# tanwanirahul/surreal

Hardware: AMD Instinct MI355X
Metric: PPO learner env-steps/sec/node (GAE+update) at 1/2/4/8 GPUs; % HBM roofline (higher is better)
Workload: dtype f32; 1 GPU; C3: synthetic PPO learner batch, reference PPO defaults (LSTM 100, horizon 5, heads 300x200, n_step 25, adapt, z-filter, 10/10 epochs), SawyerLift state dims (obs 42, act 8), 1024 segments split over 1 GPU(s) (1024 per GPU); segments_per_gpu=1024, n_step=25, env_steps_per_learn_per_gpu=25600, global_segments=1024, parallelism=single, epochs_run_last=10, ppo_mode=adapt, launch=hipGraph replay

## Files before the change

### surreal_amd/csrc/head_kernels.hip

```cpp
#include "smi_device.hpp"
#include "smi_internal.hpp"
#include "pol_rows.hpp"

namespace smi {

constexpr int HC_MAXK = 512;

struct HeadFwdArgs {
  const float* X; int64_t ldx; int K0;
  const float* W1; const float* b1;
  const float* W2; const float* b2;
  const float* W3; const float* b3;
  int h1, h2, out, tanh_out;
  float* HA1; float* HA2;
  float* Y; int64_t ldy;
  float* W1T; float* W2T;
  int64_t rows; const int* skip;
  int ld0, ld1, ld2;
  int o1, oR, shared;
  const float* vret; float* vgrad; float vscale;
  double* vpart;
};

struct HeadBwdArgs {
  const float* dZ; int out;
  const float* W3;
  const float* W2T;
  const float* W1T;
  int h1, h2, dx0, dxn;
  const float* HA1; const float* HA2;
  float* dH2; float* dH1;
  float* dX; int64_t lddx;
  const float* mask; int64_t ldm;
  int64_t rows; const int* skip;
  int ld2, ld1;
  PolRowArgs pg;
};

#ifdef SMI_PROF
__device__ unsigned long long g_head_ticks[2][10];
#define HEAD_T0() unsigned long long h_t0_ = wall_clock64(), h_prev_ = h_t0_
#define HEAD_TICK(k, id)                                                   \
  do {                                                                      \
    if (threadIdx.x == 0) {                                                 \
      const unsigned long long n_ = wall_clock64();                         \
      atomicAdd(&g_head_ticks[k][id], n_ - h_prev_);                        \
      h_prev_ = n_;                                                         \
    }                                                                       \
  } while (0)
#define HEAD_END(k)                                                        \
  do {                                                                      \
    if (threadIdx.x == 0) {                                                 \
      atomicAdd(&g_head_ticks[k][8], 1ull);                                 \
      atomicAdd(&g_head_ticks[k][9], wall_clock64() - h_t0_);               \
    }                                                                       \
  } while (0)
#else
#define HEAD_T0() (void)0
#define HEAD_TICK(k, id) (void)0
#define HEAD_END(k) (void)0
#endif

__device__ __forceinline__ void hc_sync() {
  __builtin_amdgcn_fence(__ATOMIC_RELEASE, "workgroup", "local");
  __builtin_amdgcn_s_barrier();
  __builtin_amdgcn_fence(__ATOMIC_ACQUIRE, "workgroup", "local");
}

constexpr int HC_D = 2;
constexpr int HC_XB = 4;
static_assert(HC_D >= 2, "ring of at least two chunks");
template <int NT>
struct HcStream {
  const float* wp[NT];
  float4 b[HC_D][NT];
  int K, nch, c0, cst, ntv;
  __device__ __forceinline__ void ldb(int c, float4 (&bb)[NT]) {
    const int lk = (threadIdx.x & 63) >> 4;
    const int kk = min(16 * c + 4 * lk, K - 4);
#pragma unroll
    for (int t = 0; t < NT; ++t) bb[t] = *reinterpret_cast<const float4*>(wp[t] + kk);
  }
  __device__ __forceinline__ void init(const float* __restrict__ W, int64_t ldw, int K_, int N,
                                       int nt0, int ntst, int c0_, int cst_) {
    const int li = threadIdx.x & 15;
    const int CT = (N + 15) >> 4;
    K = K_; nch = (K + 15) >> 4; c0 = c0_; cst = cst_;
    ntv = __builtin_amdgcn_readfirstlane(nt0 < CT ? (CT - 1 - nt0) / ntst + 1 : 0);
#pragma unroll
    for (int t = 0; t < NT; ++t) {
      const int n = min(16 * (nt0 + ntst * t) + li, N - 1);
      wp[t] = W + (int64_t)n * ldw;
    }
    ldb(min(c0, nch - 1), b[0]);
    ldb(min(c0 + cst, nch - 1), b[1]);
  }
};

template <int NT, int RT, bool CM = false>
__device__ __forceinline__ void hc_run(HcStream<NT>& S, const float* sA, int lda,
                                       f32x4 (&acc)[RT][NT]) {
  const int lane = threadIdx.x & 63, li = lane & 15, lk = lane >> 4;
#pragma unroll
  for (int rt = 0; rt < RT; ++rt)
#pragma unroll
    for (int t = 0; t < NT; ++t) acc[rt][t] = f32x4{0.f, 0.f, 0.f, 0.f};
  if (S.ntv == 0) return;
  const float* ap = sA + li * lda + 4 * lk;
  auto mm = [&](const float4 (&a)[RT], const float4 (&bb)[NT]) {
    if constexpr (!CM) {
#pragma unroll
      for (int t = 0; t < NT; ++t) {
#pragma unroll
        for (int rt = 0; rt < RT; ++rt) acc[rt][t] = mfma4(a[rt].x, bb[t].x, acc[rt][t]);
#pragma unroll
        for (int rt = 0; rt < RT; ++rt) acc[rt][t] = mfma4(a[rt].y, bb[t].y, acc[rt][t]);
#pragma unroll
        for (int rt = 0; rt < RT; ++rt) acc[rt][t] = mfma4(a[rt].z, bb[t].z, acc[rt][t]);
#pragma unroll
        for (int rt = 0; rt < RT; ++rt) acc[rt][t] = mfma4(a[rt].w, bb[t].w, acc[rt][t]);
      }
    } else {
#pragma unroll
      for (int t = 0; t < NT; ++t)
#pragma unroll
        for (int rt = 0; rt < RT; ++rt) acc[rt][t] = mfma4(a[rt].x, bb[t].x, acc[rt][t]);
#pragma unroll
      for (int t = 0; t < NT; ++t)
#pragma unroll
        for (int rt = 0; rt < RT; ++rt) acc[rt][t] = mfma4(a[rt].y, bb[t].y, acc[rt][t]);
#pragma unroll
      for (int t = 0; t < NT; ++t)
#pragma unroll
        for (int rt = 0; rt < RT; ++rt) acc[rt][t] = mfma4(a[rt].z, bb[t].z, acc[rt][t]);
#pragma unroll
      for (int t = 0; t < NT; ++t)
#pragma unroll
        for (int rt = 0; rt < RT; ++rt) acc[rt][t] = mfma4(a[rt].w, bb[t].w, acc[rt][t]);
    }
  };
  auto lda_ = [&](int c, float4 (&o)[RT]) {
#pragma unroll
    for (int rt = 0; rt < RT; ++rt)
      o[rt] = *reinterpret_cast<const float4*>(ap + rt * 16 * lda + 16 * c);
  };
  const int nch = S.nch, cst = S.cst, cl = nch - 1;
  int c = S.c0;
  float4 a[HC_D][RT];
#pragma unroll
  for (int d = 2; d < HC_D; ++d) S.ldb(min(c + d * cst, cl), S.b[d]);
#pragma unroll
  for (int d = 0; d < HC_D; ++d) lda_(min(c + d * cst, cl), a[d]);
  for (; c + (2 * HC_D - 1) * cst < nch; c += HC_D * cst) {
#pragma unroll
    for (int d = 0; d < HC_D; ++d) {
      mm(a[d], S.b[d]);
      lda_(c + (d + HC_D) * cst, a[d]);
      S.ldb(c + (d + HC_D) * cst, S.b[d]);
      __builtin_amdgcn_sched_barrier(0);
    }
  }
#pragma unroll
  for (int d = 0; d < HC_D; ++d) {
    if (c + d * cst < nch) mm(a[d], S.b[d]);
    lda_(min(c + (d + HC_D) * cst, cl), a[d]);
    S.ldb(min(c + (d + HC_D) * cst, cl), S.b[d]);
  }
#pragma unroll
  for (int d = 0; d < HC_D; ++d)
    if (c + (d + HC_D) * cst < nch) mm(a[d], S.b[d]);
}

template <int NT, int EPI, int RT>
__device__ __forceinline__ void hc_epi_load(int nt0, int N, const float* bias, const float* mask,
                                            int64_t r0, int64_t rows, float (&e)[RT][NT][4]) {
  const int lane = threadIdx.x & 63, li = lane & 15, lk = lane >> 4;
#pragma unroll
  for (int t = 0; t < NT; ++t) {
    const int nc = min(16 * (nt0 + 4 * t) + li, N - 1);
    if constexpr (EPI == 0) {
      e[0][t][0] = bias[nc];
    } else {
#pragma unroll
      for (int rt = 0; rt < RT; ++rt)
#pragma unroll
        for (int i = 0; i < 4; ++i) {
          const int64_t r = r0 + 16 * rt + 4 * lk + i;
          e[rt][t][i] = mask[(r < rows ? r : rows - 1) * N + nc];
        }
    }
  }
}

template <int NT, int EPI, int RT>
__device__ __forceinline__ void hc_store(const f32x4 (&acc)[RT][NT], const float (&e)[RT][NT][4],
                                         int nt0, int N, float* sO, int ldo) {
  const int lane = threadIdx.x & 63, li = lane & 15, lk = lane >> 4;
  const int CT = (N + 15) >> 4;
#pragma unroll
  for (int t = 0; t < NT; ++t) {
    const int nt = nt0 + 4 * t;
    if (nt >= CT) break;
    const int n = 16 * nt + li;
    const bool nv = n < N;
#pragma unroll
    for (int rt = 0; rt < RT; ++rt)
#pragma unroll
      for (int i = 0; i < 4; ++i) {
        const int r = 16 * rt + 4 * lk + i;
        float v;
        if constexpr (EPI == 0) {
          v = acc[rt][t][i] + e[0][t][0];
          v = v > 0.f ? v : 0.f;
        } else {
          v = e[rt][t][i] > 0.f ? acc[rt][t][i] : 0.f;
        }
        sO[r * ldo + n] = nv ? v : 0.f;
      }
  }
}

template <int RT>
__device__ __forceinline__ void hc_copy_out(const float* sO, int ld, int N, float* __restrict__ G,
                                           int64_t r0, int64_t rows) {
  if (G == nullptr) return;
  constexpr int J = HC_MAXK / 4 / 16;
  const int nq = N >> 2, q0 = threadIdx.x & 15;
#pragma unroll
  for (int rt = 0; rt < RT; ++rt) {
    const int r = (threadIdx.x >> 4) + 16 * rt;
    float4 v[J];
#pragma unroll
    for (int j = 0; j < J; ++j) {
      const int q = q0 + 16 * j;
      v[j] = q < nq ? *reinterpret_cast<const float4*>(sO + r * ld + 4 * q) : float4{0.f, 0.f, 0.f, 0.f};
    }
    if (r0 + r >= rows) continue;
    float* g = G + (r0 + r) * N;
#pragma unroll
    for (int j = 0; j < J; ++j) {
      const int q = q0 + 16 * j;
      if (q < nq) *reinterpret_cast<float4*>(g + 4 * q) = v[j];
    }
  }
}

__device__ __forceinline__ void hc_transpose_tile(const float* __restrict__ W, int M, int K,
                                                  float* __restrict__ WT, int tix, float* sT) {
  const int tk = (K + 31) >> 5;
  const int m0 = (tix / tk) * 32, k0 = (tix % tk) * 32;
  __syncthreads();
  static_assert(32 * 32 % kWG == 0, "whole tile passes");
  constexpr int TP = 32 * 32 / kWG;
  float v[TP];
#pragma unroll
  for (int i = 0; i < TP; ++i) {
    const int e = threadIdx.x + i * kWG, r = e >> 5, c = e & 31;
    v[i] = W[(int64_t)min(m0 + r, M - 1) * K + min(k0 + c, K - 1)];
  }
#pragma unroll
  for (int i = 0; i < TP; ++i) asm volatile("" : "+v"(v[i]));
#pragma unroll
  for (int i = 0; i < TP; ++i) {
    const int e = threadIdx.x + i * kWG, r = e >> 5, c = e & 31;
    if (m0 + r < M && k0 + c < K) sT[r * 33 + c] = v[i];
  }
  __syncthreads();
  for (int e = threadIdx.x; e < 32 * 32; e += kWG) {
    const int r = e >> 5, c = e & 31;
    if (k0 + r < K && m0 + c < M) WT[(int64_t)(k0 + r) * M + m0 + c] = sT[c * 33 + r];
  }
}

template <int NT1, int NT2, int RT>
__global__ void __launch_bounds__(kWG)
head_fwd_kernel(HeadFwdArgs a) {
  if (a.skip && a.skip[0] != 0) return;
  constexpr int R = HC_R * RT;
  extern __shared__ __attribute__((aligned(16))) float hsm[];
  float* s0 = hsm;
  float* s2 = hsm;
  float* s1 = hsm + a.o1;
  float* sR = hsm + a.oR;
  const int wave = __builtin_amdgcn_readfirstlane(threadIdx.x >> 6);
  const int lane = threadIdx.x & 63, li = lane & 15, lk = lane >> 4;
  const int64_t r0 = (int64_t)blockIdx.x * R;
  HEAD_T0();
  if (r0 < a.rows) {
    HcStream<NT1> S1;
    S1.init(a.W1, a.K0, a.K0, a.h1, wave, 4, 0, 1);
    float e1[RT][NT1][4];
    hc_epi_load<NT1, 0, RT>(wave, a.h1, a.b1, nullptr, r0, a.rows, e1);
    const int q0 = (a.ld0 - 4) >> 2;
    for (int e0 = threadIdx.x; e0 < R * q0; e0 += HC_XB * kWG) {
      f32x4 v[HC_XB];
#pragma unroll
      for (int k = 0; k < HC_XB; ++k) {
        const int e = min(e0 + k * kWG, R * q0 - 1);
        const int r = e / q0, q = e - r * q0;
        const int64_t rr = r0 + r < a.rows ? r0 + r : a.rows - 1;
        v[k] = *reinterpret_cast<const f32x4*>(a.X + rr * a.ldx + min(4 * q, a.K0 - 4));
      }
#pragma unroll
      for (int k = 0; k < HC_XB; ++k) {
        const int e = e0 + k * kWG;
        if (e >= R * q0) break;
        const int r = e / q0, q = e - r * q0;
        const f32x4 z = {0.f, 0.f, 0.f, 0.f};
        *reinterpret_cast<f32x4*>(s0 + r * a.ld0 + 4 * q) = 4 * q < a.K0 ? v[k] : z;
      }
    }
    __syncthreads();
    HEAD_TICK(0, 0);
    HcStream<NT2> S2;
    float e2[RT][NT2][4];
    {
      f32x4 acc[RT][NT1];
      __builtin_amdgcn_s_waitcnt(0x0F70);
      hc_run<NT1, RT>(S1, s0, a.ld0, acc);
      HEAD_TICK(0, 1);
      S2.init(a.W2, a.h1, a.h1, a.h2, wave, 4, 0, 1);
      hc_epi_load<NT2, 0, RT>(wave, a.h2, a.b2, nullptr, r0, a.rows, e2);
      if constexpr (RT == 2) {
        if (a.shared) hc_sync();
      }
      hc_store<NT1, 0, RT>(acc, e1, wave, a.h1, s1, a.ld1);
    }
    hc_sync();
    HEAD_TICK(0, 2);
    hc_copy_out<RT>(s1, a.ld1, a.h1, a.HA1, r0, a.rows);
    HEAD_TICK(0, 3);
    HcStream<1> S3;
    {
      f32x4 acc[RT][NT2];
      hc_run<NT2, RT>(S2, s1, a.ld1, acc);
      HEAD_TICK(0, 4);
      S3.init(a.W3, a.h2, a.h2, a.out, 0, 1, wave, 4);
      if constexpr (RT == 2) {
        if (a.shared) hc_sync();
      }
      hc_store<NT2, 0, RT>(acc, e2, wave, a.h2, s2, a.ld2);
    }
    hc_sync();
    HEAD_TICK(0, 5);
    hc_copy_out<RT>(s2, a.ld2, a.h2, a.HA2, r0, a.rows);
    {
      const float bn = a.b3[li < a.out ? li : a.out - 1];
      float vr[RT][4];
      if (a.vgrad) {
#pragma unroll
        for (int rt = 0; rt < RT; ++rt)
#pragma unroll
          for (int i = 0; i < 4; ++i)
            vr[rt][i] = a.vret[min(r0 + 16 * rt + 4 * lk + i, a.rows - 1)];
      }
      f32x4 acc[RT][1];
      hc_run<1, RT>(S3, s2, a.ld2, acc);
#pragma unroll
      for (int rt = 0; rt < RT; ++rt)
        *reinterpret_cast<float4*>(sR + ((wave * RT + rt) * 64 + lane) * 4) =
            float4{acc[rt][0][0], acc[rt][0][1], acc[rt][0][2], acc[rt][0][3]};
      hc_sync();
      double vs[5] = {0.0, 0.0, 0.0, 0.0, 0.0};
      if (wave == 0 && li < a.out) {
        __builtin_amdgcn_s_waitcnt(0x0F70);
#pragma unroll
        for (int rt = 0; rt < RT; ++rt)
#pragma unroll
          for (int i = 0; i < 4; ++i) {
            const int r = 16 * rt + 4 * lk + i;
            if (r0 + r >= a.rows) continue;
            const float v = ((sR[((0 * RT + rt) * 64 + lane) * 4 + i] + sR[((1 * RT + rt) * 64 + lane) * 4 + i]) +
                             (sR[((2 * RT + rt) * 64 + lane) * 4 + i] + sR[((3 * RT + rt) * 64 + lane) * 4 + i])) + bn;
            const float y = a.tanh_out ? tanhf(v) : v;
            a.Y[(r0 + r) * a.ldy + li] = y;
            if (a.vgrad) {
              const float rv = vr[rt][i];
              a.vgrad[r0 + r] = a.vscale * (y - rv);
              if (a.vpart) {
                const float e = y - rv;
                const double dd = (double)rv - (double)y;
                vs[0] += (double)(e * e);
                vs[1] += dd; vs[2] += dd * dd;
                vs[3] += (double)rv; vs[4] += (double)rv * (double)rv;
              }
            }
          }
      }
      if (a.vpart && wave == 0) {
#pragma unroll
        for (int k = 0; k < 5; ++k) {
          const double t = wave_sum_d(vs[k]);
          if (lane == 0) a.vpart[(int64_t)blockIdx.x * 5 + k] = t;
        }
      }
    }
  }
  HEAD_TICK(0, 6);
  if (a.W1T) {
    const int t1 = ((a.h1 + 31) >> 5) * ((a.K0 + 31) >> 5);
    const int t2 = ((a.h2 + 31) >> 5) * ((a.h1 + 31) >> 5);
    for (int tix = blockIdx.x; tix < t1 + t2; tix += gridDim.x) {
      if (tix < t1) hc_transpose_tile(a.W1, a.h1, a.K0, a.W1T, tix, sR);
      else hc_transpose_tile(a.W2, a.h2, a.h1, a.W2T, tix - t1, sR);
    }
  }
  HEAD_TICK(0, 7);
  HEAD_END(0);
}

static_assert(sizeof(PolGradShared) <= HC_PG_LDS, "head_plan counts the prologue's static LDS");
template <int NTA, int NTB, int RT, bool PG>
__global__ void __launch_bounds__(kWG, RT == 1 ? 3 : 2)
head_bwd_kernel(HeadBwdArgs a) {
  if (a.skip && a.skip[0] != 0) return;
  constexpr int R = HC_R * RT;
  extern __shared__ __attribute__((aligned(16))) float hsm[];
  float* s2 = hsm;
  float* s1 = s2 + R * a.ld2;
  float* sZ = s1 + R * a.ld1;
  const int wave = __builtin_amdgcn_readfirstlane(threadIdx.x >> 6);
  const int lane = threadIdx.x & 63, li = lane & 15, lk = lane >> 4;
  const int64_t r0 = (int64_t)blockIdx.x * R;
  const int out = a.out;
  HEAD_T0();
  const int zr = threadIdx.x >> 4, zk = threadIdx.x & 15;
  HcStream<NTA> SA;
  if constexpr (PG) {
    constexpr int AT = 8;
    __shared__ PolGradShared psh;
    const int t = threadIdx.x;
    const int64_t n = r0 + t;
    const bool own = t < R && n < a.rows;
    PolGradRow<AT> x;
    if (own) x.load(a.pg, n, AT);
    SA.init(a.W2T, a.h2, a.h2, a.h1, wave, 4, 0, 1);
    float wsurr, wkl;
    PolGradPre pre;
    if (pol_grad_weights<1>(a.pg, psh, wsurr, wkl, pre)) return;
    const PolGradCols<AT> cols(pre, psh, AT);
    const AdvNorm nadv(a.pg, pre.mom);
    float glv[AT];
#pragma unroll
    for (int j = 0; j < AT; ++j) glv[j] = 0.f;
    if (t < R) {
      float dz[AT];
      if (own) {
        pol_grad_compute<AT>(a.pg, cols, nadv, x, wsurr, wkl, dz, glv);
        st_row<AT>(a.pg.dz + n * AT, dz, AT);
      } else {
#pragma unroll
        for (int j = 0; j < AT; ++j) dz[j] = 0.f;
      }
#pragma unroll
      for (int j = 0; j < 16; ++j) sZ[t * 16 + j] = j < AT ? dz[j] : 0.f;
    }
    if (wave == 0) {
#pragma unroll
      for (int j = 0; j < AT; ++j) {
        const float sg = wave_sum(glv[j]);
        if (lane == 0) a.pg.lvpart[(int64_t)blockIdx.x * AT + j] = sg;
      }
    }
  } else {
    float zv[RT];
#pragma unroll
    for (int rt = 0; rt < RT; ++rt)
      zv[rt] = a.dZ[min(r0 + 16 * rt + zr, a.rows - 1) * out + min(zk, out - 1)];
    SA.init(a.W2T, a.h2, a.h2, a.h1, wave, 4, 0, 1);
#pragma unroll
    for (int rt = 0; rt < RT; ++rt) sZ[(16 * rt + zr) * 16 + zk] = zk < out ? zv[rt] : 0.f;
  }
  const int h2p = a.ld2 - 4;
  for (int e = threadIdx.x; e < R * (h2p - a.h2); e += kWG) {
    const int r = e / (h2p - a.h2), c = e - r * (h2p - a.h2);
    s2[r * a.ld2 + a.h2 + c] = 0.f;
  }
  __syncthreads();
  const int nq = a.h2 >> 2;
#pragma unroll
  for (int q0 = 0; q0 < 128; q0 += 64) {
    if (q0 >= nq) break;
    const bool qv = q0 + lane < nq;
    const int q = qv ? q0 + lane : nq - 1;
    constexpr int KGM = 4;
    f32x4 w[KGM][4], m[RT][4];
#pragma unroll
    for (int g = 0; g < KGM; ++g)
#pragma unroll
      for (int j = 0; j < 4; ++j)
        w[g][j] = *reinterpret_cast<const f32x4*>(a.W3 + (int64_t)min(4 * g + j, out - 1) * a.h2 + 4 * q);
#pragma unroll
    for (int rt = 0; rt < RT; ++rt)
#pragma unroll
      for (int i = 0; i < 4; ++i) {
        const int64_t rr = min(r0 + 16 * rt + 4 * wave + i, a.rows - 1);
        m[rt][i] = *reinterpret_cast<const f32x4*>(a.HA2 + rr * a.h2 + 4 * q);
      }
#pragma unroll
    for (int rt = 0; rt < RT; ++rt) {
      f32x4 v[4];
#pragma unroll
      for (int i = 0; i < 4; ++i) v[i] = f32x4{0.f, 0.f, 0.f, 0.f};
#pragma unroll
      for (int g = 0; g < KGM; ++g) {
        if (4 * g >= out) break;
#pragma unroll
        for (int j = 0; j < 4; ++j)
#pragma unroll
          for (int i = 0; i < 4; ++i) {
            const float z = sZ[(16 * rt + 4 * wave + i) * 16 + 4 * g + j];
            v[i][0] = fmaf(z, w[g][j][0], v[i][0]); v[i][1] = fmaf(z, w[g][j][1], v[i][1]);
            v[i][2] = fmaf(z, w[g][j][2], v[i][2]); v[i][3] = fmaf(z, w[g][j][3], v[i][3]);
          }
      }
#pragma unroll
      for (int i = 0; i < 4; ++i) {
        const int r = 16 * rt + 4 * wave + i;
        const f32x4 o = {m[rt][i][0] > 0.f ? v[i][0] : 0.f, m[rt][i][1] > 0.f ? v[i][1] : 0.f,
                         m[rt][i][2] > 0.f ? v[i][2] : 0.f, m[rt][i][3] > 0.f ? v[i][3] : 0.f};
        if (qv) {
          *reinterpret_cast<f32x4*>(s2 + r * a.ld2 + 4 * q) = o;
          if (r0 + r < a.rows) *reinterpret_cast<f32x4*>(a.dH2 + (r0 + r) * a.h2 + 4 * q) = o;
        }
      }
    }
  }
  float eA[RT][NTA][4];
  hc_epi_load<NTA, 1, RT>(wave, a.h1, nullptr, a.HA1, r0, a.rows, eA);
  hc_sync();
  HEAD_TICK(1, 0);
  HcStream<NTB> SB;
  {
    f32x4 acc[RT][NTA];
    hc_run<NTA, RT, true>(SA, s2, a.ld2, acc);
    HEAD_TICK(1, 1);
    if (a.dxn > 0)
      SB.init(a.W1T + (int64_t)a.dx0 * a.h1, a.h1, a.h1, a.dxn, wave, 4, 0, 1);
    hc_store<NTA, 1, RT>(acc, eA, wave, a.h1, s1, a.ld1);
  }
  hc_sync();
  HEAD_TICK(1, 2);
  hc_copy_out<RT>(s1, a.ld1, a.h1, a.dH1, r0, a.rows);
  HEAD_TICK(1, 3);
  if (a.dxn <= 0) { HEAD_END(1); return; }
  {
    f32x4 acc[RT][NTB];
    hc_run<NTB, RT, true>(SB, s1, a.ld1, acc);
    HEAD_TICK(1, 4);
    const int CT = (a.dxn + 15) >> 4;
#pragma unroll
    for (int t = 0; t < NTB; ++t) {
      const int nt = wave + 4 * t;
      if (nt >= CT) break;
      const int n = 16 * nt + li;
      if (n >= a.dxn) continue;
#pragma unroll
      for (int rt = 0; rt < RT; ++rt)
#pragma unroll
        for (int i = 0; i < 4; ++i) {
          const int64_t r = r0 + 16 * rt + 4 * lk + i;
          if (r >= a.rows) continue;
          float v = acc[rt][t][i];
          if (a.mask) v = a.mask[r * a.ldm + n] > 0.f ? v : 0.f;
          a.dX[r * a.lddx + n] = v;
        }
    }
  }
  HEAD_TICK(1, 5);
  HEAD_END(1);
}

#ifdef SMI_PROF
extern "C" int smi_head_phase_ticks(unsigned long long* out ) {
  if (hipMemcpyFromSymbol(out, HIP_SYMBOL(g_head_ticks), sizeof(g_head_ticks)) != hipSuccess)
    return SMI_E_LAUNCH;
  static const unsigned long long zero[20] = {};
  return hipMemcpyToSymbol(HIP_SYMBOL(g_head_ticks), zero, sizeof(zero)) == hipSuccess ? SMI_OK
                                                                                        : SMI_E_LAUNCH;
}
#endif

static bool al16(const void* p) { return (reinterpret_cast<uintptr_t>(p) & 15) == 0; }

bool head_fused_ok(int in, int64_t ldx, int h1, int h2, int out, const float* X,
                   const float* W1, const float* W2, const float* W3) {
  return in >= 4 && in <= 320 && in % 4 == 0 && ldx % 4 == 0 &&
         h1 >= 4 && h1 <= HC_MAXK && h1 % 4 == 0 && h2 >= 4 && h2 <= HC_MAXK && h2 % 4 == 0 &&
         out >= 1 && out <= 16 && al16(X) && al16(W1) && al16(W2) && al16(W3);
}


int launch_head_fwd_fused(const float* X, int64_t ldx, int64_t rows, int in, const float* W1,
                          const float* b1, int h1, const float* W2, const float* b2, int h2,
                          const float* W3, const float* b3, int out, int tanh_out, float* HA1,
                          float* HA2, float* Y, int64_t ldy, float* W1T, float* W2T,
                          hipStream_t st, const int* skip, const float* vret, float* vgrad,
                          float vscale, double* vpart) {
  if (rows <= 0) return SMI_OK;
  if (vgrad && (out != 1 || !vret)) return set_error(SMI_E_ARG, "head_forward: value epilogue needs out == 1");
  if (vpart && !vgrad) return set_error(SMI_E_ARG, "head_forward: value statistics need the value epilogue");
  const HeadPlan hp = head_plan(rows, in, h1, h2, 0);
  HeadFwdArgs a{X, ldx, in, W1, b1, W2, b2, W3, b3, h1, h2, out, tanh_out, HA1, HA2, Y, ldy,
                W1T, W2T, rows, skip, hp.ld0, hp.ld1, hp.ld2, hp.fwd_o1, hp.fwd_oR, hp.fwd_shared,
                vret, vgrad, vscale};
  a.vpart = vpart;
  const int rt = hp.rt;
  const size_t lds = (size_t)hp.fwd_lds;
  const dim3 grid((unsigned)hp.grid);
  const int m1 = hp.fwd_n1, n2 = hp.fwd_n2;
  const int kslot = ktime_begin(st);
  const char* form = "head_fwd_kernel";
#define SMI_HF(A, B)                                                                    \
  do {                                                                                  \
    if (rt == 2) {                                                                      \
      allow_lds(head_fwd_kernel<A, B, 2>, lds);                                         \
      hipLaunchKernelGGL((head_fwd_kernel<A, B, 2>), grid, dim3(kWG), lds, st, a);      \
      form = "head_fwd_kernel<" #A "," #B ",rt2>";                                      \
    } else {                                                                            \
      allow_lds(head_fwd_kernel<A, B, 1>, lds);                                         \
      hipLaunchKernelGGL((head_fwd_kernel<A, B, 1>), grid, dim3(kWG), lds, st, a);      \
      form = "head_fwd_kernel<" #A "," #B ",rt1>";                                      \
    }                                                                                   \
  } while (0)
#define SMI_HF2(A)                                        \
  do {                                                    \
    switch (n2) {                                         \
      case 2: SMI_HF(A, 2); break;                        \
      case 3: SMI_HF(A, 3); break;                        \
      case 4: SMI_HF(A, 4); break;                        \
      case 5: SMI_HF(A, 5); break;                        \
      default: SMI_HF(A, 8); break;                       \
    }                                                     \
  } while (0)
  if (m1 == 2) SMI_HF2(2);
  else if (m1 == 5) SMI_HF2(5);
  else SMI_HF2(8);
#undef SMI_HF2
#undef SMI_HF
  ktime_end(kslot, KT_GEMM_FWD,
            2.0 * (double)rows * ((double)in * h1 + (double)h1 * h2 + (double)h2 * out), st);
  return check_launch(form);
}

int launch_head_bwd_fused(const float* dZ, int out, int64_t rows, const float* W3,
                          const float* W2T, const float* W1T, int h1, int h2, int dx0, int dxn,
                          const float* HA1, const float* HA2, float* dH2, float* dH1, float* dX,
                          int64_t lddx, const float* mask, int64_t ldm, hipStream_t st,
                          const int* skip, const PolRowArgs* pg) {
  if (rows <= 0) return SMI_OK;
  if (pg && out != 8) return set_error(SMI_E_ARG, "head_backward: the policy prologue needs out == 8");
  const HeadPlan hp = head_plan(rows, 0, h1, h2, dxn);
  HeadBwdArgs a{dZ, out, W3, W2T, W1T, h1, h2, dx0, dxn, HA1, HA2, dH2, dH1, dX, lddx, mask, ldm,
                rows, skip, hp.ld2, hp.ld1};
  if (pg) a.pg = *pg;
  const int rt = hp.rt;
  const size_t lds = (size_t)hp.bwd_lds;
  const dim3 grid((unsigned)hp.grid);
  const int na = hp.bwd_na, nb = hp.bwd_nb;
  const int kslot = ktime_begin(st);
  const char* form = "head_bwd_kernel";
#define SMI_HB2(A, B, P)                                                               \
  do {                                                                                 \
    if (rt == 2) {                                                                     \
      allow_lds(head_bwd_kernel<A, B, 2, P>, lds);                                     \
      hipLaunchKernelGGL((head_bwd_kernel<A, B, 2, P>), grid, dim3(kWG), lds, st, a);  \
      form = P ? "head_bwd_kernel<" #A "," #B ",rt2,pg>" : "head_bwd_kernel<" #A "," #B ",rt2>"; \
    } else {                                                                           \
      allow_lds(head_bwd_kernel<A, B, 1, P>, lds);                                     \
      hipLaunchKernelGGL((head_bwd_kernel<A, B, 1, P>), grid, dim3(kWG), lds, st, a);  \
      form = P ? "head_bwd_kernel<" #A "," #B ",rt1,pg>" : "head_bwd_kernel<" #A "," #B ",rt1>"; \
    }                                                                                  \
  } while (0)
#define SMI_HB(A, B)                                                                   \
  do {                                                                                 \
    if (pg) SMI_HB2(A, B, true);                                                       \
    else SMI_HB2(A, B, false);                                                         \
  } while (0)
  if (na == 2 && nb == 2) SMI_HB(2, 2);
  else if (na == 2) SMI_HB(2, 5);
  else if (na == 5 && nb == 2) SMI_HB(5, 2);
  else if (na == 5) SMI_HB(5, 5);
  else if (nb == 2) SMI_HB(8, 2);
  else SMI_HB(8, 5);
#undef SMI_HB
#undef SMI_HB2
  ktime_end(kslot, KT_GEMM_DX,
            2.0 * (double)rows * ((double)out * h2 + (double)h2 * h1 + (double)h1 * dxn), st);
  return check_launch(form);
}

}
```

Baseline: 3.990 million env-steps/s.

## Specialize head MFMA bodies by live tile count and hoist W3 loads early

Weight stream pointers become 32-bit byte offsets from a single base, which cuts per-tile address registers. The MFMA loop body is templated on the number of valid column tiles, and hc_run dispatches at runtime to a version that skips MFMAs and loads for tiles a wave does not own. In the backward head, the dz·W3 step is templated on the output-group count, so small action dims use fewer weight registers. W3 and HA2 loads are issued before the barrier in the RT==2/NTA==5 case so they overlap with the policy-gradient prologue. The cost is more code instantiations and possibly higher register pressure from the values held across the barrier.

Result: faster. 4.134 million env-steps/s, median of 6 (+3.6%).

```diff
diff --git a/surreal_amd/csrc/head_kernels.hip b/surreal_amd/csrc/head_kernels.hip
--- a/surreal_amd/csrc/head_kernels.hip
+++ b/surreal_amd/csrc/head_kernels.hip
@@ -1,6 +1,7 @@
 #include "smi_device.hpp"
 #include "smi_internal.hpp"
 #include "pol_rows.hpp"
+#include <type_traits>
 
 namespace smi {
 
@@ -72,45 +73,42 @@
 static_assert(HC_D >= 2, "ring of at least two chunks");
 template <int NT>
 struct HcStream {
-  const float* wp[NT];
+  const float* W;
+  unsigned wo[NT];
   float4 b[HC_D][NT];
   int K, nch, c0, cst, ntv;
+  template <int NV = NT>
   __device__ __forceinline__ void ldb(int c, float4 (&bb)[NT]) {
     const int lk = (threadIdx.x & 63) >> 4;
-    const int kk = min(16 * c + 4 * lk, K - 4);
-#pragma unroll
-    for (int t = 0; t < NT; ++t) bb[t] = *reinterpret_cast<const float4*>(wp[t] + kk);
-  }
-  __device__ __forceinline__ void init(const float* __restrict__ W, int64_t ldw, int K_, int N,
+    const unsigned kb = 4u * (unsigned)min(16 * c + 4 * lk, K - 4);
+#pragma unroll
+    for (int t = 0; t < NV; ++t)
+      bb[t] = *reinterpret_cast<const float4*>(reinterpret_cast<const char*>(W) + (size_t)(wo[t] + kb));
+  }
+  __device__ __forceinline__ void init(const float* __restrict__ W_, int ldw, int K_, int N,
                                        int nt0, int ntst, int c0_, int cst_) {
     const int li = threadIdx.x & 15;
     const int CT = (N + 15) >> 4;
-    K = K_; nch = (K + 15) >> 4; c0 = c0_; cst = cst_;
+    W = W_; K = K_; nch = (K + 15) >> 4; c0 = c0_; cst = cst_;
     ntv = __builtin_amdgcn_readfirstlane(nt0 < CT ? (CT - 1 - nt0) / ntst + 1 : 0);
 #pragma unroll
     for (int t = 0; t < NT; ++t) {
       const int n = min(16 * (nt0 + ntst * t) + li, N - 1);
-      wp[t] = W + (int64_t)n * ldw;
+      wo[t] = 4u * (unsigned)(n * ldw);
     }
     ldb(min(c0, nch - 1), b[0]);
     ldb(min(c0 + cst, nch - 1), b[1]);
   }
 };
 
-template <int NT, int RT, bool CM = false>
-__device__ __forceinline__ void hc_run(HcStream<NT>& S, const float* sA, int lda,
-                                       f32x4 (&acc)[RT][NT]) {
-  const int lane = threadIdx.x & 63, li = lane & 15, lk = lane >> 4;
-#pragma unroll
-  for (int rt = 0; rt < RT; ++rt)
-#pragma unroll
-    for (int t = 0; t < NT; ++t) acc[rt][t] = f32x4{0.f, 0.f, 0.f, 0.f};
-  if (S.ntv == 0) return;
-  const float* ap = sA + li * lda + 4 * lk;
+template <int NT, int NV, int RT, bool CM>
+__device__ __forceinline__ void hc_body(HcStream<NT>& S, const float* ap, int lda,
+                                        f32x4 (&acc)[RT][NT]) {
+  static_assert(NV >= 1 && NV <= NT, "a body for 1 .. NT tiles");
   auto mm = [&](const float4 (&a)[RT], const float4 (&bb)[NT]) {
     if constexpr (!CM) {
 #pragma unroll
-      for (int t = 0; t < NT; ++t) {
+      for (int t = 0; t < NV; ++t) {
 #pragma unroll
         for (int rt = 0; rt < RT; ++rt) acc[rt][t] = mfma4(a[rt].x, bb[t].x, acc[rt][t]);
 #pragma unroll
@@ -122,19 +120,19 @@
       }
     } else {
 #pragma unroll
-      for (int t = 0; t < NT; ++t)
+      for (int t = 0; t < NV; ++t)
 #pragma unroll
         for (int rt = 0; rt < RT; ++rt) acc[rt][t] = mfma4(a[rt].x, bb[t].x, acc[rt][t]);
 #pragma unroll
-      for (int t = 0; t < NT; ++t)
+      for (int t = 0; t < NV; ++t)
 #pragma unroll
         for (int rt = 0; rt < RT; ++rt) acc[rt][t] = mfma4(a[rt].y, bb[t].y, acc[rt][t]);
 #pragma unroll
-      for (int t = 0; t < NT; ++t)
+      for (int t = 0; t < NV; ++t)
 #pragma unroll
         for (int rt = 0; rt < RT; ++rt) acc[rt][t] = mfma4(a[rt].z, bb[t].z, acc[rt][t]);
 #pragma unroll
-      for (int t = 0; t < NT; ++t)
+      for (int t = 0; t < NV; ++t)
 #pragma unroll
         for (int rt = 0; rt < RT; ++rt) acc[rt][t] = mfma4(a[rt].w, bb[t].w, acc[rt][t]);
     }
@@ -148,7 +146,7 @@
   int c = S.c0;
   float4 a[HC_D][RT];
 #pragma unroll
-  for (int d = 2; d < HC_D; ++d) S.ldb(min(c + d * cst, cl), S.b[d]);
+  for (int d = 2; d < HC_D; ++d) S.template ldb<NV>(min(c + d * cst, cl), S.b[d]);
 #pragma unroll
   for (int d = 0; d < HC_D; ++d) lda_(min(c + d * cst, cl), a[d]);
   for (; c + (2 * HC_D - 1) * cst < nch; c += HC_D * cst) {
@@ -156,7 +154,7 @@
     for (int d = 0; d < HC_D; ++d) {
       mm(a[d], S.b[d]);
       lda_(c + (d + HC_D) * cst, a[d]);
-      S.ldb(c + (d + HC_D) * cst, S.b[d]);
+      S.template ldb<NV>(c + (d + HC_D) * cst, S.b[d]);
       __builtin_amdgcn_sched_barrier(0);
     }
   }
@@ -164,11 +162,31 @@
   for (int d = 0; d < HC_D; ++d) {
     if (c + d * cst < nch) mm(a[d], S.b[d]);
     lda_(min(c + (d + HC_D) * cst, cl), a[d]);
-    S.ldb(min(c + (d + HC_D) * cst, cl), S.b[d]);
+    S.template ldb<NV>(min(c + (d + HC_D) * cst, cl), S.b[d]);
   }
 #pragma unroll
   for (int d = 0; d < HC_D; ++d)
     if (c + (d + HC_D) * cst < nch) mm(a[d], S.b[d]);
+}
+
+template <int NT, int RT, bool CM = false, bool EX = true>
+__device__ __forceinline__ void hc_run(HcStream<NT>& S, const float* sA, int lda,
+                                       f32x4 (&acc)[RT][NT]) {
+  const int lane = threadIdx.x & 63, li = lane & 15, lk = lane >> 4;
+#pragma unroll
+  for (int rt = 0; rt < RT; ++rt)
+#pragma unroll
+    for (int t = 0; t < NT; ++t) acc[rt][t] = f32x4{0.f, 0.f, 0.f, 0.f};
+  if (S.ntv == 0) return;
+  const float* ap = sA + li * lda + 4 * lk;
+  constexpr int N1 = NT > 1 ? NT - 1 : 1, N2 = NT > 2 ? NT - 2 : N1;
+  if constexpr (NT == 1 || !EX) {
+    hc_body<NT, NT, RT, CM>(S, ap, lda, acc);
+  } else {
+    if (S.ntv >= NT) hc_body<NT, NT, RT, CM>(S, ap, lda, acc);
+    else if (N2 == N1 || S.ntv >= N1) hc_body<NT, N1, RT, CM>(S, ap, lda, acc);
+    else hc_body<NT, N2, RT, CM>(S, ap, lda, acc);
+  }
 }
 
 template <int NT, int EPI, int RT>
@@ -317,7 +335,7 @@
     {
       f32x4 acc[RT][NT1];
       __builtin_amdgcn_s_waitcnt(0x0F70);
-      hc_run<NT1, RT>(S1, s0, a.ld0, acc);
+      hc_run<NT1, RT, false, RT == 2>(S1, s0, a.ld0, acc);
       HEAD_TICK(0, 1);
       S2.init(a.W2, a.h1, a.h1, a.h2, wave, 4, 0, 1);
       hc_epi_load<NT2, 0, RT>(wave, a.h2, a.b2, nullptr, r0, a.rows, e2);
@@ -333,7 +351,7 @@
     HcStream<1> S3;
     {
       f32x4 acc[RT][NT2];
-      hc_run<NT2, RT>(S2, s1, a.ld1, acc);
+      hc_run<NT2, RT, false, RT == 2>(S2, s1, a.ld1, acc);
       HEAD_TICK(0, 4);
       S3.init(a.W3, a.h2, a.h2, a.out, 0, 1, wave, 4);
       if constexpr (RT == 2) {
@@ -425,106 +443,151 @@
   const int out = a.out;
   HEAD_T0();
   const int zr = threadIdx.x >> 4, zk = threadIdx.x & 15;
+  const int nq = a.h2 >> 2;
   HcStream<NTA> SA;
+  constexpr bool EARLY = RT == 2 && NTA == 5;
+  PolGradShared* pshp = nullptr;
   if constexpr (PG) {
-    constexpr int AT = 8;
     __shared__ PolGradShared psh;
-    const int t = threadIdx.x;
-    const int64_t n = r0 + t;
-    const bool own = t < R && n < a.rows;
-    PolGradRow<AT> x;
-    if (own) x.load(a.pg, n, AT);
-    SA.init(a.W2T, a.h2, a.h2, a.h1, wave, 4, 0, 1);
-    float wsurr, wkl;
-    PolGradPre pre;
-    if (pol_grad_weights<1>(a.pg, psh, wsurr, wkl, pre)) return;
-    const PolGradCols<AT> cols(pre, psh, AT);
-    const AdvNorm nadv(a.pg, pre.mom);
-    float glv[AT];
-#pragma unroll
-    for (int j = 0; j < AT; ++j) glv[j] = 0.f;
-    if (t < R) {
-      float dz[AT];
-      if (own) {
-        pol_grad_compute<AT>(a.pg, cols, nadv, x, wsurr, wkl, dz, glv);
-        st_row<AT>(a.pg.dz + n * AT, dz, AT);
-      } else {
-#pragma unroll
-        for (int j = 0; j < AT; ++j) dz[j] = 0.f;
-      }
-#pragma unroll
-      for (int j = 0; j < 16; ++j) sZ[t * 16 + j] = j < AT ? dz[j] : 0.f;
-    }
-    if (wave == 0) {
-#pragma unroll
-      for (int j = 0; j < AT; ++j) {
-        const float sg = wave_sum(glv[j]);
-        if (lane == 0) a.pg.lvpart[(int64_t)blockIdx.x * AT + j] = sg;
-      }
-    }
-  } else {
-    float zv[RT];
+    pshp = &psh;
+  }
+  float zv[RT];
+  if constexpr (!PG) {
 #pragma unroll
     for (int rt = 0; rt < RT; ++rt)
       zv[rt] = a.dZ[min(r0 + 16 * rt + zr, a.rows - 1) * out + min(zk, out - 1)];
     SA.init(a.W2T, a.h2, a.h2, a.h1, wave, 4, 0, 1);
-#pragma unroll
-    for (int rt = 0; rt < RT; ++rt) sZ[(16 * rt + zr) * 16 + zk] = zk < out ? zv[rt] : 0.f;
-  }
-  const int h2p = a.ld2 - 4;
-  for (int e = threadIdx.x; e < R * (h2p - a.h2); e += kWG) {
-    const int r = e / (h2p - a.h2), c = e - r * (h2p - a.h2);
-    s2[r * a.ld2 + a.h2 + c] = 0.f;
-  }
-  __syncthreads();
-  const int nq = a.h2 >> 2;
-#pragma unroll
-  for (int q0 = 0; q0 < 128; q0 += 64) {
-    if (q0 >= nq) break;
-    const bool qv = q0 + lane < nq;
-    const int q = qv ? q0 + lane : nq - 1;
-    constexpr int KGM = 4;
-    f32x4 w[KGM][4], m[RT][4];
-#pragma unroll
-    for (int g = 0; g < KGM; ++g)
-#pragma unroll
-      for (int j = 0; j < 4; ++j)
-        w[g][j] = *reinterpret_cast<const f32x4*>(a.W3 + (int64_t)min(4 * g + j, out - 1) * a.h2 + 4 * q);
-#pragma unroll
-    for (int rt = 0; rt < RT; ++rt)
-#pragma unroll
-      for (int i = 0; i < 4; ++i) {
-        const int64_t rr = min(r0 + 16 * rt + 4 * wave + i, a.rows - 1);
-        m[rt][i] = *reinterpret_cast<const f32x4*>(a.HA2 + rr * a.h2 + 4 * q);
-      }
-#pragma unroll
-    for (int rt = 0; rt < RT; ++rt) {
-      f32x4 v[4];
-#pragma unroll
-      for (int i = 0; i < 4; ++i) v[i] = f32x4{0.f, 0.f, 0.f, 0.f};
-#pragma unroll
-      for (int g = 0; g < KGM; ++g) {
-        if (4 * g >= out) break;
+  }
+  auto dz_w3 = [&](auto kgc) -> bool {
+    constexpr int KG = decltype(kgc)::value;
+    f32x4 w[KG][4], m[RT][4];
+    auto ldwm = [&](int q) {
+#pragma unroll
+      for (int g = 0; g < KG; ++g)
 #pragma unroll
         for (int j = 0; j < 4; ++j)
-#pragma unroll
-          for (int i = 0; i < 4; ++i) {
-            const float z = sZ[(16 * rt + 4 * wave + i) * 16 + 4 * g + j];
-            v[i][0] = fmaf(z, w[g][j][0], v[i][0]); v[i][1] = fmaf(z, w[g][j][1], v[i][1]);
-            v[i][2] = fmaf(z, w[g][j][2], v[i][2]); v[i][3] = fmaf(z, w[g][j][3], v[i][3]);
+          w[g][j] = *reinterpret_cast<const f32x4*>(a.W3 + (int64_t)min(4 * g + j, out - 1) * a.h2 + 4 * q);
+#pragma unroll
+      for (int rt = 0; rt < RT; ++rt)
+#pragma unroll
+        for (int i = 0; i < 4; ++i) {
+          const int64_t rr = min(r0 + 16 * rt + 4 * wave + i, a.rows - 1);
+          m[rt][i] = *reinterpret_cast<const f32x4*>(a.HA2 + rr * a.h2 + 4 * q);
+        }
+    };
+    auto fma_store = [&](bool qv, int q) {
+#pragma unroll
+      for (int rt = 0; rt < RT; ++rt) {
+        f32x4 v[4];
+#pragma unroll
+        for (int i = 0; i < 4; ++i) v[i] = f32x4{0.f, 0.f, 0.f, 0.f};
+#pragma unroll
+        for (int g = 0; g < KG; ++g) {
+          if (4 * g >= out) break;
+#pragma unroll
+          for (int j = 0; j < 4; ++j)
+#pragma unroll
+            for (int i = 0; i < 4; ++i) {
+              const float z = sZ[(16 * rt + 4 * wave + i) * 16 + 4 * g + j];
+              v[i][0] = fmaf(z, w[g][j][0], v[i][0]); v[i][1] = fmaf(z, w[g][j][1], v[i][1]);
+              v[i][2] = fmaf(z, w[g][j][2], v[i][2]); v[i][3] = fmaf(z, w[g][j][3], v[i][3]);
+            }
+        }
+#pragma unroll
+        for (int i = 0; i < 4; ++i) {
+          const int r = 16 * rt + 4 * wave + i;
+          const f32x4 o = {m[rt][i][0] > 0.f ? v[i][0] : 0.f, m[rt][i][1] > 0.f ? v[i][1] : 0.f,
+                           m[rt][i][2] > 0.f ? v[i][2] : 0.f, m[rt][i][3] > 0.f ? v[i][3] : 0.f};
+          if (qv) {
+            *reinterpret_cast<f32x4*>(s2 + r * a.ld2 + 4 * q) = o;
+            if (r0 + r < a.rows) *reinterpret_cast<f32x4*>(a.dH2 + (r0 + r) * a.h2 + 4 * q) = o;
           }
-      }
-#pragma unroll
-      for (int i = 0; i < 4; ++i) {
-        const int r = 16 * rt + 4 * wave + i;
-        const f32x4 o = {m[rt][i][0] > 0.f ? v[i][0] : 0.f, m[rt][i][1] > 0.f ? v[i][1] : 0.f,
-                         m[rt][i][2] > 0.f ? v[i][2] : 0.f, m[rt][i][3] > 0.f ? v[i][3] : 0.f};
-        if (qv) {
-          *reinterpret_cast<f32x4*>(s2 + r * a.ld2 + 4 * q) = o;
-          if (r0 + r < a.rows) *reinterpret_cast<f32x4*>(a.dH2 + (r0 + r) * a.h2 + 4 * q) = o;
-        }
-      }
-    }
+        }
+      }
+    };
+    const bool qv0 = lane < nq;
+    const int qa = qv0 ? lane : nq - 1;
+    if constexpr (PG) {
+      constexpr int AT = 8;
+      PolGradShared& psh = *pshp;
+      const int t = threadIdx.x;
+      const int64_t n = r0 + t;
+      const bool own = t < R && n < a.rows;
+      PolGradRow<AT> x;
+      if (own) x.load(a.pg, n, AT);
+      SA.init(a.W2T, a.h2, a.h2, a.h1, wave, 4, 0, 1);
+      if constexpr (EARLY) ldwm(qa);
+      float wsurr, wkl;
+      PolGradPre pre;
+      if (pol_grad_weights<1>(a.pg, psh, wsurr, wkl, pre)) return true;
+      const PolGradCols<AT> cols(pre, psh, AT);
+      const AdvNorm nadv(a.pg, pre.mom);
+      float glv[AT];
+#pragma unroll
+      for (int j = 0; j < AT; ++j) glv[j] = 0.f;
+      if (t < R) {
+        float dz[AT];
+        if (own) {
+          pol_grad_compute<AT>(a.pg, cols, nadv, x, wsurr, wkl, dz, glv);
+          st_row<AT>(a.pg.dz + n * AT, dz, AT);
+        } else {
+#pragma unroll
+          for (int j = 0; j < AT; ++j) dz[j] = 0.f;
+        }
+#pragma unroll
+        for (int j = 0; j < 16; ++j) sZ[t * 16 + j] = j < AT ? dz[j] : 0.f;
+      }
+      if (wave == 0) {
+#pragma unroll
+        for (int j = 0; j < AT; ++j) {
+          const float sg = wave_sum(glv[j]);
+          if (lane == 0) a.pg.lvpart[(int64_t)blockIdx.x * AT + j] = sg;
+        }
+      }
+    } else {
+      if constexpr (EARLY) ldwm(qa);
+#pragma unroll
+      for (int rt = 0; rt < RT; ++rt) sZ[(16 * rt + zr) * 16 + zk] = zk < out ? zv[rt] : 0.f;
+    }
+    const int h2p = a.ld2 - 4;
+    for (int e = threadIdx.x; e < R * (h2p - a.h2); e += kWG) {
+      const int r = e / (h2p - a.h2), c = e - r * (h2p - a.h2);
+      s2[r * a.ld2 + a.h2 + c] = 0.f;
+    }
+    __syncthreads();
+    if constexpr (EARLY) {
+#pragma unroll
+      for (int g = 0; g < KG; ++g)
+#pragma unroll
+        for (int j = 0; j < 4; ++j) asm volatile("" : "+v"(w[g][j]));
+#pragma unroll
+      for (int rt = 0; rt < RT; ++rt)
+#pragma unroll
+        for (int i = 0; i < 4; ++i) asm volatile("" : "+v"(m[rt][i]));
+    } else {
+      ldwm(qa);
+    }
+    fma_store(qv0, qa);
+    if (nq > 64) {
+      const bool qv = 64 + lane < nq;
+      const int q = qv ? 64 + lane : nq - 1;
+      ldwm(q);
+      fma_store(qv, q);
+    }
+    return false;
+  };
+  {
+    bool stop;
+    if constexpr (PG) {
+      stop = dz_w3(std::integral_constant<int, 2>{});
+    } else if constexpr (!EARLY) {
+      stop = dz_w3(std::integral_constant<int, 4>{});
+    } else {
+      if (out <= 4) stop = dz_w3(std::integral_constant<int, 1>{});
+      else if (out <= 8) stop = dz_w3(std::integral_constant<int, 2>{});
+      else stop = dz_w3(std::integral_constant<int, 4>{});
+    }
+    if (stop) return;
   }
   float eA[RT][NTA][4];
   hc_epi_load<NTA, 1, RT>(wave, a.h1, nullptr, a.HA1, r0, a.rows, eA);
@@ -533,7 +596,7 @@
   HcStream<NTB> SB;
   {
     f32x4 acc[RT][NTA];
-    hc_run<NTA, RT, true>(SA, s2, a.ld2, acc);
+    hc_run<NTA, RT, true, (RT == 2 && NTA < 8)>(SA, s2, a.ld2, acc);
     HEAD_TICK(1, 1);
     if (a.dxn > 0)
       SB.init(a.W1T + (int64_t)a.dx0 * a.h1, a.h1, a.h1, a.dxn, wave, 4, 0, 1);
@@ -546,7 +609,7 @@
   if (a.dxn <= 0) { HEAD_END(1); return; }
   {
     f32x4 acc[RT][NTB];
-    hc_run<NTB, RT, true>(SB, s1, a.ld1, acc);
+    hc_run<NTB, RT, true, RT == 2>(SB, s1, a.ld1, acc);
     HEAD_TICK(1, 4);
     const int CT = (a.dxn + 15) >> 4;
 #pragma unroll
```
